# garg02/mpi-sppy

Measured on AMD Instinct MI355X. Metric: PH scenario-iterations/sec (farmer 100k) + time to conv<1e-4, higher is better.
Workload: dtype f64; 1 GPU; farmer crops_multiplier=1, 100000 scenarios (BASELINE configs[2]); scenarios=100000, scenarios_per_gpu=100000, n=12, m=7, nonants=3, parallelism=scenario-sharded x1, RCCL allreduce

## Files before the change

### mpi-sppy_amd/csrc/phx_jit.h

```cpp
#pragma once
#include <stdint.h>
#include <math.h>
#include <stdio.h>
#include <algorithm>
#include <sstream>
#include <string>
#include <vector>
#include "phx_setup.h"

namespace phx {

struct LaneStructure {
    int n = 0, m = 0, nnz = 0, npairs = 0, nvar = 0, nslot = 0;
    bool c_vary = false, bnd_vary = false, rhs_vary = false;
    bool scaled = false;
    std::vector<int32_t> row, col, kvar, col_slot;
    std::vector<int32_t> pair_a, pair_b, pair_pos;
    std::vector<uint8_t> lnz;
    std::vector<uint8_t> rfirst, cfirst, rempty, cempty;
    std::vector<uint8_t> lfin, ufin, fixed, blfin, bufin, eq;
    std::vector<double> Ac, dc, dr, c, lb, ub, bl, bu;
    double ipm_xs = 1.0, ipm_zs = 1.0, ipm_ws = 1.0;
    double multi_theta = 0.0;
    int multi_rounds = 0;
// ... 241 lines not shown
         "  phx_lane::lane_stamp(io, 1);\n"
         "  const int t = blockIdx.x * 64 + threadIdx.x;\n"
         "  bool still = false;\n"
         "  if (t < io.S) {\n"
         "    phx_lane::lane_stamp(io, 2);\n"
         "    still = " + wl + "(io, t);\n"
         "  }\n"
         "  phx_lane::lane_stamp(io, 3);\n"
         "  phx_lane::compact_lane(still, t, io.lanes_out, io.count_out);\n"
         "  phx_lane::lane_stamp(io, 4);\n"
         "  phx_lane::lane_stamp(io, 5);\n"
         "}\n";
    o << "extern \"C\" __global__ void __launch_bounds__(64, 1) phx_lane_warm_fz1(phx_lane::LaneIO io) {\n"
         "  phx_lane::warm_fused<PT>(io);\n"
         "}\n";
    o << "extern \"C\" __global__ void __launch_bounds__(64, 2) phx_lane_warm_fzr2(phx_lane::LaneIO io) {\n"
         "  phx_lane::warm_fused<PT, PHX_FZR2_CARRY_DEF, PHX_FZR2_PARK_DEF>(io);\n"
         "}\n";
    o << "extern \"C\" __global__ void __launch_bounds__(64, 1) phx_lane_all(phx_lane::LaneIO io, int rescue) {\n"
         "  if (phx_lane::gated(io.gate)) return;\n"
         "  phx_lane::zero_next_counts(io.counts_next);\n"
         "  const int t = blockIdx.x * 64 + threadIdx.x;\n"
         "  bool still = false;\n"
         "  if (t < io.S) still = phx_lane::all_lane<PT>(io, t, rescue);\n"
         "  phx_lane::compact_lane(still, t, io.lanes_out, io.count_out);\n"
         "}\n";
    o << "extern \"C\" __global__ void __launch_bounds__(64, 1) phx_lane_all_rl(phx_lane::LaneIO io, int rescue) {\n"
         "  if (phx_lane::gated(io.gate)) return;\n"
         "  phx_lane::zero_next_counts(io.counts_next);\n"
         "  const int t = blockIdx.x * 64 + threadIdx.x;\n"
         "  bool still = false;\n"
         "  if (t < io.S) still = phx_lane::all_lane<PT, false>(io, t, rescue);\n"
         "  phx_lane::compact_lane(still, t, io.lanes_out, io.count_out);\n"
         "}\n";
    o << "extern \"C\" __global__ void __launch_bounds__(64, 1) phx_lane_all_pk(phx_lane::LaneIO io, int rescue) {\n"
         "  __shared__ double pk[phx_lane::Data<PT>::PARK * 64];\n"
         "  if (phx_lane::gated(io.gate)) return;\n"
         "  phx_lane::zero_next_counts(io.counts_next);\n"
         "  const int t = blockIdx.x * 64 + threadIdx.x;\n"
         "  bool still = false;\n"
         "  if (t < io.S) still = phx_lane::all_lane<PT, false, true>(io, t, rescue, pk);\n"
         "  phx_lane::compact_lane(still, t, io.lanes_out, io.count_out);\n"
         "}\n";
    o << "extern \"C\" __global__ void __launch_bounds__(64) phx_fz_tail(phx_lane::LaneIO io, phx_lane::TailCopy tc) {\n"
         "  phx_lane::fz_tail<PT>(io, tc);\n"
         "}\n";
    o << "extern \"C\" __global__ void __launch_bounds__(64, 4) phx_lane_map(phx_lane::LaneIO io) {\n"
         "  if (phx_lane::gated(io.gate)) return;\n"
         "  phx_lane::zero_next_counts(io.counts_next);\n"
         "  const int t = blockIdx.x * 64 + threadIdx.x;\n"
         "  bool still = false;\n"
         "  if (t < io.S) still = phx_lane::map_lane<PT>(io, t);\n"
         "  phx_lane::compact_lane(still, t, io.lanes_out, io.count_out);\n"
         "}\n";
    const std::string wlr = with_map ? "phx_lane::warm_lane<PT, true, true>" : "phx_lane::warm_lane<PT, false, true>";
    o << "#ifdef PHX_LIST_RELOAD\n#define PHX_LIST_WAVES " << warm_waves << "\n#define PHX_LIST_FN " << wl
      << "\n#else\n#define PHX_LIST_WAVES 1\n#define PHX_LIST_FN " << wlr << "\n#endif\n";
    o << "extern \"C\" __global__ void __launch_bounds__(64, PHX_LIST_WAVES"
      << ") phx_lane_warm_list(phx_lane::LaneIO io, const int* lanes, const int* count) {\n"
// ... 59 lines not shown
```

### mpi-sppy_amd/csrc/phx_kernels.hip

```cpp
#include <hip/hip_runtime.h>
#include <stdio.h>
#include <string.h>
#include <math.h>
#include <string>
#include <vector>
#include <algorithm>
#include "../../include/phx.h"
#include "phx_core.h"
#include "phx_setup.h"
#include "phx_wg.h"
#include "phx_sp.h"
#include "phx_jit.h"
#include "phx_lane.h"
#include <hip/hiprtc.h>
#include <rccl/rccl.h>
#include <map>
#include <memory>
#include <mutex>
#include <stdlib.h>
#include <atomic>
#include <chrono>

#include "phx_lane_src.inc"

// ... 781 lines not shown
    int lane_ww = 2, lane_cw = 1;
    std::string lane_defs;
    LaneMod mod_ph, mod_fix;
    bool fix_built = false;
    bool fix_ok = false;
    bool fix_lane = false;
    double *fix_lb = nullptr, *fix_ub = nullptr;
    bool ovr_base_ok = false;
    const double* fix_vals = nullptr;
    const int32_t* fix_idx = nullptr;
    LaneMod mod_sub;
    std::vector<uint8_t> sub_mask;
    bool sub_ok = false;
    bool sub_lane = false;
    std::string sub_info;
    mutable std::string jit_text;
    const int32_t* fix_where = nullptr;
    const double *raw_lb = nullptr, *raw_ub = nullptr;
    int64_t raw_si = 0, raw_ss = 0;
    int32_t* fixer_new = nullptr;
    int32_t* donor_dev = nullptr;
    int donor_cap = 0;
    std::vector<int32_t> donor_lo, donor_hi;
    const void* donor_key[3] = {nullptr, nullptr, nullptr};
    int donor_key_n[2] = {0, 0};
    const double *ph_W = nullptr, *ph_rho = nullptr, *ph_xbar = nullptr;
    const int32_t* ph_idx = nullptr;
    int32_t ph_W_on = 0, ph_prox_on = 0;
    bool ph_dirty = false;
    int32_t* counts = nullptr;
// ... 72 lines not shown
#define PHX_CHECK(ctx, expr)                                                      \
    do {                                                                          \
        hipError_t _e = (expr);                                                   \
        if (_e != hipSuccess) {                                                   \
            (ctx)->err = std::string(#expr) + ": " + hipGetErrorString(_e);       \
            return 1;                                                             \
        }                                                                         \
    } while (0)

#define PHX_REQUIRE(ctx, cond, msg)                                               \
    do {                                                                          \
        if (!(cond)) { (ctx)->err = (msg); return 1; }                            \
    } while (0)

static inline unsigned nblk(int64_t n, int b) { return (unsigned)((n + b - 1) / b); }

static int ev_index(const phx_ctx* c, hipEvent_t e) {
    const hipEvent_t evs[5] = {c->ev0, c->ev1, c->ev2, c->ev3, c->ev4};
    for (int k = 0; k < 5; ++k)
        if (e && e == evs[k]) return k;
    return -1;
}

static hipError_t ev_record(phx_ctx* c, hipEvent_t e, hipStream_t st) {
    const hipError_t r = hipEventRecord(e, st);
    const int k = ev_index(c, e);
    if (r == hipSuccess && k >= 0) c->run.ev_rec |= 1u << k;
    return r;
}

// ... 544 lines not shown
                {
                    const size_t NS = (size_t)std::max(ctx->N, 1) * S;
                    ctx->lane_zero_d = ctx->alloc<double>(NS);
                    ctx->lane_zero_i = ctx->alloc<int32_t>(NS);
                    PHX_REQUIRE(ctx, ctx->lane_zero_d != nullptr && ctx->lane_zero_i != nullptr,
                                "phx_set_problem: out of device memory (lane stand-ins)");
                    PHX_CHECK(ctx, hipMemset(ctx->lane_zero_d, 0, sizeof(double) * NS));
                    PHX_CHECK(ctx, hipMemset(ctx->lane_zero_i, 0, sizeof(int32_t) * NS));
                }
                ctx->seed_buf = ctx->alloc<int32_t>(2 * SEED_T + 2);
                ctx->seed_aset = ctx->alloc<uint32_t>((size_t)SEED_T * phx_lane::aset_words(n, m));
                PHX_REQUIRE(ctx, ctx->aset != nullptr && ctx->seed_buf != nullptr,
                            "phx_set_problem: out of device memory (aset)");
                PHX_CHECK(ctx, hipMemset(ctx->aset, 0, sizeof(uint32_t) * nw));
                if (getenv("PHX_LANE_STAMPS") && atoi(getenv("PHX_LANE_STAMPS")) == 1) {
                    const size_t ns = (size_t)nblk(S, PHX_BLOCK) * 8;
                    ctx->lane_stamps = ctx->alloc<uint64_t>(ns);
                    if (ctx->lane_stamps) PHX_CHECK(ctx, hipMemset(ctx->lane_stamps, 0, sizeof(uint64_t) * ns));
                }
                if (want_map) {
                    ctx->lane_map = ctx->alloc<double>(mw * S);
                    PHX_REQUIRE(ctx, ctx->lane_map != nullptr, "phx_set_problem: out of device memory (map)");
                }
            }
        } else {
            ctx->jit_info = "off: " + why;
        }
    }
    hipLaunchKernelGGL(k_norm_init, dim3(nblk(S, PHX_BLOCK)), dim3(PHX_BLOCK), 0, 0, St, S);
    if (launch_begin(ctx, 0, 0, nullptr)) return 1;
    PHX_CHECK(ctx, hipGetLastError());
// ... 715 lines not shown
    io.status_out = status_out; io.iters_out = iters_out;
    io.max_it = o->ipm_max_it; io.ipm_tol = o->lane_ipm_tol > 0 ? o->lane_ipm_tol : o->ipm_tol; io.kkt_tol = o->kkt_tol; io.reg = o->reg;
    io.refine = o->refine_steps;
    io.as_rounds = o->as_rounds > 0 ? o->as_rounds : 1;
    io.single_after = 3;
    io.gate = gate;
    io.map = ctx->lane_map;
    io.fz = phx_lane::FusedW{};
    io.counts_next = nullptr;
    io.stamps = ctx->lane_stamps;
    return io;
}

static void report_lane_stamps(phx_ctx* ctx) {
    if (!ctx->lane_stamps) return;
    const unsigned G = nblk(ctx->S, PHX_BLOCK);
    std::vector<uint64_t> h((size_t)G * 8);
    if (hipMemcpy(h.data(), ctx->lane_stamps, sizeof(uint64_t) * h.size(), hipMemcpyDeviceToHost) != hipSuccess)
        return;
    uint64_t t0 = ~0ull, tend = 0, last_start = 0, first_end = ~0ull;
    double ph[5] = {0, 0, 0, 0, 0}, life = 0.0, lmax = 0.0;
    int nw = 0;
    for (unsigned b = 0; b < G; ++b) {
        const uint64_t* s = h.data() + (size_t)b * 8;
        if (!s[0] || !s[5] || s[5] < s[0]) continue;
        t0 = std::min(t0, s[0]);
        tend = std::max(tend, s[5]);
        last_start = std::max(last_start, s[0]);
        first_end = std::min(first_end, s[5]);
        for (int k = 0; k < 5; ++k) ph[k] += (double)(s[k + 1] - s[k]);
        life += (double)(s[5] - s[0]);
// ... 26 lines not shown
            const uint64_t* s = h.data() + (size_t)b * 8;
            if (!s[0] || !s[5] || s[5] < s[0] || s[5] < s[4]) continue;
            arr.emplace_back(s[4], b);
        }
        std::sort(arr.begin(), arr.end());
        const size_t n = arr.size(), nl = std::min<size_t>(n, 8);
        double ep_all = 0.0, ep_last = 0.0;
        for (size_t i = 0; i < n; ++i) {
            const uint64_t* s = h.data() + (size_t)arr[i].second * 8;
            ep_all += (double)(s[5] - s[4]);
            if (i + nl >= n) ep_last = std::max(ep_last, (double)(s[5] - s[4]));
        }
        if (n) {
            const uint64_t* sl = h.data() + (size_t)arr[n - 1].second * 8;
            fprintf(stderr,
                    "[lane stamps] by arrival at the epilogue: last arrival +%.2f us (block %u), its epilogue %.2f us; "
                    "launch end %.2f us after the last arrival; epilogue mean %.2f us, longest among the last %d "
                    "arrivals %.2f us\n",
                    (arr[n - 1].first - t0) * 0.01, arr[n - 1].second, (sl[5] - sl[4]) * 0.01,
                    (tend - arr[n - 1].first) * 0.01, ep_all / n * 0.01, (int)nl, ep_last * 0.01);
        }
    }
    fprintf(stderr,
            "[lane stamps] waves %d span %.2f us, last start +%.2f us, first end +%.2f us; per wave lifetime "
            "%.2f us (max %.2f): prologue %.2f, update_w %.2f, solve %.2f, compact %.2f, epilogue %.2f us\n",
            nw, (tend - t0) * 0.01, (last_start - t0) * 0.01, (first_end - t0) * 0.01, life / nw * 0.01, lmax * 0.01,
            ph[0] / nw * 0.01, ph[1] / nw * 0.01, ph[2] / nw * 0.01, ph[3] / nw * 0.01, ph[4] / nw * 0.01);
    (void)hipMemset(ctx->lane_stamps, 0, sizeof(uint64_t) * h.size());
}

static int rescue_rounds(const phx_solve_opts* o) {
// ... 44 lines not shown
        void* wargs[] = {&io};
        PHX_CHECK(ctx, hipModuleLaunchKernel(ctx->lane_warm_fn, G, 1, 1, PHX_BLOCK, 1, 1, 0, st, wargs, nullptr));
    }
    PHX_CHECK(ctx, hipGetLastError());
    io.counts_next = nullptr;
    io.lanes_out = ctx->lanesB;
    io.count_out = C + 1;
    io.as_rounds = std::max(io.as_rounds, rescue_rounds(o));
    const int32_t* in_l = ctx->lanesA;
    const int32_t* in_c = C;
    if (launch_cold(ctx, io, in_l, in_c, Gl, st)) return 1;
    *npass_out = 1;
    return 0;
}

static hipFunction_t fused_kernel(const phx_ctx* ctx, unsigned G) {
    static const bool fzr2_off = getenv("PHX_FZR2") && atoi(getenv("PHX_FZR2")) == 0;
    return (!fzr2_off && (int64_t)G > (int64_t)ctx->simds) ? ctx->lane_warm_fzr2_fn : ctx->lane_warm_fz1_fn;
}

static int enqueue_lane_solve(phx_ctx* ctx, const phx_solve_opts* o, hipStream_t st, int32_t* C, double* x_out,
                              double* y_out, double* obj_out, int32_t* status_out, int32_t* iters_out,
                              const int32_t* gate, hipEvent_t ev_a, hipEvent_t ev_b, hipEvent_t ev_c,
                              int* npass_out, unsigned cold_blocks = 0,
                              const phx_lane::FusedW* fz = nullptr, int mode = 0) {
    const int S = ctx->S;
    const unsigned G = nblk(S, PHX_BLOCK);
    phx_lane::LaneIO io = lane_io(ctx, o, x_out, y_out, obj_out, status_out, iters_out, gate);
    io.fz = fz ? *fz : phx_lane::FusedW{};
    if (fz) io.xbar_node = fz->stage;
    const bool warm_as = ctx->have_aset && o->as_rounds > 0 && ctx->lane_warm_fn;
    const bool use_map = ctx->lane_map != nullptr && ctx->lane_map_fn != nullptr;
    int npass = warm_as ? (use_map ? 2 : std::max(1, std::min(o->warm_passes, 8))) : 0;
// ... 11 lines not shown
        PHX_CHECK(ctx, hipModuleLaunchKernel(ctx->lane_all_fn, G, 1, 1, PHX_BLOCK, 1, 1, 0, st, aargs, nullptr));
        if (ev_b) PHX_CHECK(ctx, ev_record(ctx, ev_b, st));
        *npass_out = 0;
        return 0;
    }
    const unsigned Gl = std::min<unsigned>(G, 1024u);
    const unsigned Gc = cold_blocks ? std::min<unsigned>(G, cold_blocks) : Gl;
    if (ev_a) PHX_CHECK(ctx, ev_record(ctx, ev_a, st));
    for (int k = 0; k < npass && mode != 2; ++k) {
        io.lanes_out = L[k & 1]; io.count_out = C + k;
        io.counts_next = k == 0 ? next : nullptr;
        io.warm_rounds = use_map ? (k == 0 ? 0 : o->as_rounds) : (npass > 1 ? 1 : o->as_rounds);
        if (k == 0) {
            void* wargs[] = {&io};
            hipFunction_t fn = use_map ? ctx->lane_map_fn : (fz ? fused_kernel(ctx, G) : ctx->lane_warm_fn);
            PHX_CHECK(ctx, hipModuleLaunchKernel(fn, G, 1, 1, PHX_BLOCK, 1, 1, 0, st, wargs, nullptr));
            if (ev_b) PHX_CHECK(ctx, ev_record(ctx, ev_b, st));
        } else {
            const int32_t* in_l = L[(k - 1) & 1];
            const int32_t* in_c = C + k - 1;
            void* largs[] = {&io, &in_l, &in_c};
            PHX_CHECK(ctx, hipModuleLaunchKernel(ctx->lane_warm_list_fn, Gl, 1, 1, PHX_BLOCK, 1, 1, 0, st,
                                                 largs, nullptr));
        }
    }
    if (npass == 0 && ev_b) PHX_CHECK(ctx, ev_record(ctx, ev_b, st));
    *npass_out = npass;
    if (mode == 1) return 0;

    io.fz = phx_lane::FusedW{};
    if (mode == 2) io.xbar_node = ctx->ph_xbar;
// ... 580 lines not shown
        return 1;
    }
    ctx->comm_ranks = nranks;
    ctx->comm_rank = rank;
    return 0;
}

int phx_last_solve_stats(const phx_ctx* ctx, phx_solve_stats* out) {
    if (!ctx || !out) return 1;
    *out = ctx->stats;
    return 0;
}

const char* phx_jit_info(const phx_ctx* ctx) {
    if (!ctx) return "null context";
    ctx->jit_text = ctx->jit_info + ctx->sub_info;
    return ctx->jit_text.c_str();
}

int phx_debug_spd_inverse(const double* s_host, int32_t ma, double* inv_host) {
    if (!s_host || !inv_host || ma < 1 || ma > WG_BLK_MAX) return -1;
    const int ld = ma | 1;
    double* d = nullptr;
    int32_t* f = nullptr;
    if (hipMalloc(&d, sizeof(double) * (size_t)ma * ld) != hipSuccess) return -1;
    if (hipMalloc(&f, sizeof(int32_t)) != hipSuccess) { (void)hipFree(d); return -1; }
    std::vector<double> h((size_t)ma * ld, 0.0);
    for (int i = 0; i < ma; ++i)
        for (int j = 0; j <= i; ++j) h[(size_t)i * ld + j] = s_host[(size_t)i * ma + j];
    int rc = 0;
    if (hipMemcpy(d, h.data(), sizeof(double) * h.size(), hipMemcpyHostToDevice) != hipSuccess) rc = -1;
// ... 337 lines not shown
        fprintf(stderr, "[iterk] S=%d lane_mode=%d wg=%d sp=%d fused=%d (fz_env %d tail %d warm %d nnodes %d NNS %d N %d "
                "ntiles %d cover %d gseg %d segs_ok %d stage_len %d need %d W %d rho %d map %d passes %d as_rounds %d) "
                "depth %d max_iters %d\n", S, (int)lane_mode, (int)wg_mode, (int)sp_mode, (int)fused, (int)fz_env,
                ctx->lane_tail_fn != nullptr, ctx->lane_warm_fn != nullptr, T->nnodes, NNS, ctx->N, T->ntiles,
                T->nnodes_cover, gseg, (int)segs_ok, a->node_stage_len, 2 * NNS + 1 + a->conv_R,
                (int)(ctx->ph_W == a->W), (int)(ctx->ph_rho == a->rho), (int)use_map, o->warm_passes, o->as_rounds,
                depth, a->max_iters);
    struct OutSet { double *x, *y, *obj; int32_t *status, *iters; };
    OutSet X[2] = {{a->x, a->y, a->obj, a->status, a->iters}, {}};
    if (fused) {
        X[1] = OutSet{ctx->alt_x, a->y ? ctx->alt_y : nullptr, ctx->alt_obj, a->status ? ctx->alt_status : nullptr,
                      a->iters ? ctx->alt_iters : nullptr};
    } else {
        X[1] = X[0];
    }
    auto make_fz = [&](int k, bool first) {
        phx_lane::FusedW f{};
        f.on = 1;
        f.iter = k;
        f.first = first ? 1 : 0;
        f.from_shards = (!first && !multi) ? 1 : 0;
        f.fold_top = multi ? 1 : 0;
        f.nb = (int32_t)nblk(S, PHX_BLOCK);
        f.stage = stage;
        f.node_sums = a->node_sums;
        f.nns = NNS;
        f.x_prev = X[(k - 1) & 1].x;
        f.pc = a->prob_coeff;
        f.ctl = ctx->ctl;
        f.prog = ctx->prog_dev;
        f.part = ctx->fz_part;
        f.tk = ctx->tickets + 2 * TICKET_SET;
        f.g = gseg;
        f.R = a->conv_R;
        f.cnt = ctx->conv_cnt_dev;
        f.thresh = a->convthresh;
        return f;
    };
// ... 178 lines not shown
                        phx_lane::TailCopy tc{};
                        if (!tail_enq) {
                            tc.left_dst = (int32_t*)ctx->tail_dev;
                            tc.left_src = C;
                            if (a->seg_sums) {
                                tc.seg_dst = a->seg_sums;
                                tc.seg_src = stage + 2 * NNS + 1;
                                tc.nseg = a->conv_R;
                            }
                        }
                        if (iter0_exp && !adopt_pending && !iter0_exp_copied) {
                            tc.exp_dst = ctx->tail_dev + 1;
                            tc.exp_src = a->iter0_expect;
                        }
                        void* targs[] = {&tio, &tc};
                        PHX_CHECK(ctx, hipModuleLaunchKernel(ctx->lane_tail_fn, 1, 1, 1, PHX_BLOCK, 1, 1, 0, st,
                                                             targs, nullptr));
                        if (tc.left_dst) {
                            tail_enq = left_in_tail = true;
                            if (tc.seg_dst) seg_copied = true;
                        }
                        if (tc.exp_dst) iter0_exp_copied = exp_in_tail = true;
                    }
                    enq.push_back(Enq{C, npass, false});
                    k_enq = k;
                    continue;
                }
                const OutSet& xin = X[(k - 1) & 1];
                const OutSet& xout = X[k & 1];
                if (small_xw) {
                    IterkCtl ic{};
                    ic.ctl = ctx->ctl;
// ... 282 lines not shown
```

### mpi-sppy_amd/csrc/phx_lane.h

```cpp
#pragma once
#if !defined(__HIPCC_RTC__)
#include <stdint.h>
#include <math.h>
#if defined(__HIPCC__)
#include <hip/hip_runtime.h>
#endif
#else
typedef long long int64_t;
typedef int int32_t;
typedef unsigned int uint32_t;
typedef unsigned long long uint64_t;
#endif

#if defined(__HIPCC__) || defined(__HIPCC_RTC__)
#define PHX_LD __host__ __device__ __forceinline__
#define PHX_UNROLL _Pragma("unroll")
#define PHX_NOUNROLL _Pragma("nounroll")
#else
#define PHX_LD inline
#define PHX_UNROLL
#define PHX_NOUNROLL
#endif
#ifdef PHX_IPM_PASS_ROLLED
#define PHX_IPM_PASS_LOOP PHX_NOUNROLL
// ... 54 lines not shown
constexpr int32_t FLAG_WRITTEN = 2;
constexpr int32_t FLAG_MAP = 4;

struct IterkProgress {
    uint64_t word;
    double conv;
};

struct FusedW {
    int32_t on;
    int32_t iter;
    int32_t first;
    int32_t from_shards;
    int32_t fold_top;
    int32_t nb;
    double* stage;
    double* node_sums;
    int32_t nns;
    const double* x_prev;
    const double* pc;
    int32_t* ctl;
    IterkProgress* prog;
    double* part;
    unsigned int* tk;
    int32_t g, R;
    const double* cnt;
    double thresh;
};

struct LaneIO {
// ... 43 lines not shown
    FusedW fz;
    uint64_t* stamps;
};

struct TailCopy {
    int32_t* left_dst;
    const int32_t* left_src;
    double* seg_dst;
    const double* seg_src;
    int32_t nseg;
    double* exp_dst;
    const double* exp_src;
};

#if defined(__HIPCC__) || defined(__HIPCC_RTC__)
__device__ __forceinline__ void lane_stamp(const LaneIO& io, int k) {
    if (io.stamps && threadIdx.x == 0) io.stamps[(uint64_t)blockIdx.x * 8 + k] = wall_clock64();
}
#endif

#if (defined(__HIPCC__) || defined(__HIPCC_RTC__)) && !defined(PHX_OUT_PLAIN)
#define PHX_OUT(lv, v) __hip_atomic_store(&(lv), (v), __ATOMIC_RELAXED, __HIP_MEMORY_SCOPE_AGENT)
#else
#define PHX_OUT(lv, v) ((lv) = (v))
#endif

PHX_LD bool gated(const int32_t* gate) { return gate && *(const volatile int32_t*)gate; }

PHX_LD void opaque(double& v) {
#if defined(__HIP_DEVICE_COMPILE__) || defined(__HIPCC_RTC__)
    __asm__ volatile("" : "+v"(v));
#else
// ... 1549 lines not shown
            *(volatile int32_t*)f.ctl = 1;
        }
        publish_progress(f.prog, it, done ? 1 : 0, conv);
    }
    return done;
}

__device__ __forceinline__ double* fz_part_set(const FusedW& f, int np, int it) {
    return f.part + (int64_t)(it & 1) * ((int64_t)f.nb + TICKET_SHARDS) * np;
}
template <int NP>
__device__ __forceinline__ void fz_shard_load(const FusedW& f, int it, double* r) {
    const unsigned nsh = (unsigned)f.nb < TICKET_SHARDS ? (unsigned)f.nb : TICKET_SHARDS;
    const double* sp = fz_part_set(f, NP, it) + (int64_t)f.nb * NP;
    PHX_UNROLL for (int u = 0; u < (TICKET_SHARDS * NP + 63) / 64; ++u) {
        const unsigned i = 64u * u + threadIdx.x;
        r[u] = i < nsh * NP ? load_wt(sp + i) : 0.0;
    }
}
template <int NP>
__device__ __forceinline__ double fz_shard_sum(const double* r, int e) {
    double a = 0.0;
    PHX_UNROLL for (int q = 0; q < TICKET_SHARDS; ++q) a += lane_get(r[(q * NP + e) / 64], (q * NP + e) % 64);
    return a;
}
template <class PT>
__device__ __forceinline__ void fz_inputs(const FusedW& f, const double* sv, double* in) {
    constexpr int NS = PT::nslot() > 0 ? PT::nslot() : 1;
    constexpr int NP = 2 * NS + 2;
    if (f.from_shards) {
        PHX_UNROLL for (int e = 0; e < NP; ++e) in[e] = fz_shard_sum<NP>(sv, e);
    } else {
        PHX_UNROLL for (int e = 0; e < NP; ++e) in[e] = 0.0;
        PHX_UNROLL for (int t = 0; t < PT::nslot(); ++t) {
            in[t] = f.stage[t];
            in[NS + t] = f.stage[f.nns + t];
        }
        in[2 * NS] = f.stage[2 * f.nns + 1 + f.g];
        in[2 * NS + 1] = f.stage[2 * f.nns];
    }
}
template <int NS>
__device__ __forceinline__ void fz_store_stage(const FusedW& f, const double* in) {
    PHX_UNROLL for (int t = 0; t < NS; ++t) {
        f.stage[t] = in[t];
        f.stage[f.nns + t] = in[NS + t];
// ... 85 lines not shown
    const int e = threadIdx.x;
    if (e < NV) {
        double a = 0.0;
        for (unsigned q = 0; q < nsh; ++q) a += load_wt(&shard_part[q * NP + e]);
        if (e < NS) f.stage[e] = a;
        else if (e < 2 * NS) f.stage[f.nns + (e - NS)] = a;
        else {
            for (int r = 0; r < f.R; ++r) f.stage[2 * f.nns + 1 + r] = r == f.g ? a : 0.0;
            f.stage[2 * f.nns] =
                (double)__hip_atomic_load(io.count_out, __ATOMIC_RELAXED, __HIP_MEMORY_SCOPE_AGENT);
        }
    }
}

template <class PT>
__device__ void fz_tail(const LaneIO& io, const TailCopy& tc) {
    const FusedW& f = io.fz;
    constexpr int NS = PT::nslot() > 0 ? PT::nslot() : 1;
    constexpr int NP = 2 * NS + 2;
    double sv[(TICKET_SHARDS * NP + 63) / 64], in[NP];
    fz_shard_load<NP>(f, f.iter, sv);
    const bool run = !gated(io.gate);
    const bool fold = run && !f.fold_top;
    PHX_UNROLL for (int e = 0; e < NP; ++e) in[e] = fz_shard_sum<NP>(sv, e);
    if (fold) {
        if (threadIdx.x == 0) fz_store_stage<NS>(f, in);
        if (tc.seg_dst)
            for (int g = threadIdx.x; g < tc.nseg; g += (int)blockDim.x) tc.seg_dst[g] = g == f.g ? in[2 * NS] : 0.0;
    }
    tail_copy(tc, !fold);
    if (!run) return;
    (void)fz_decide(f, f.iter, fz_conv(f, in[2 * NS], fold ? nullptr : f.stage + 2 * f.nns + 1));
}

template <class PT>
__device__ void seed_block(const LaneIO& io, const int32_t* tl, int T, const uint32_t* tmpl) {
    constexpr int NC = seed_coords<PT>();
    constexpr int TS = seed_templates_staged<PT>() > 0 ? seed_templates_staged<PT>() : 1;
    constexpr int NCP = NC > 0 ? NC : 1;
// ... 38 lines not shown
    for (int w = 0; w < nw; ++w) io.aset[(int64_t)w * io.S + sc] = tmpl[(int64_t)best * nw + w];
}

__device__ __forceinline__ void zero_next_counts(int32_t* next) {
    if (next && blockIdx.x == 0 && threadIdx.x < 16) next[threadIdx.x] = 0;
}

__device__ __forceinline__ void compact_lane(bool still, int sc, int32_t* out, int32_t* count) {
    const unsigned long long b = __ballot(still);
    const int lane = threadIdx.x & 63;
    int base = 0;
    if (lane == 0 && b) base = atomicAdd(count, (int32_t)__popcll(b));
    base = __shfl(base, 0, 64);
    if (still) out[base + __popcll(b & ((1ull << lane) - 1ull))] = sc;
}
template <class PT, bool CARRY = PHX_CARRY_DEF, bool PARK = false>
__device__ __forceinline__ void warm_fused(const LaneIO& io) {
    const FusedW& f = io.fz;
    constexpr int NS = PT::nslot() > 0 ? PT::nslot() : 1;
    constexpr int NP = 2 * NS + 2;
    constexpr int NVA = PT::NMAX_V, NW = aset_words(PT::NMAX_N, PT::NMAX_M);
    const int sc = blockIdx.x * 64 + threadIdx.x;
    const bool live = sc < io.S;
    const int s = live ? sc : 0;
    const int64_t S = io.S;
    double av[NVA], xv[NS], wv[NS], rv[NS], pcv[NS];
    uint32_t aw[NW];
    PHX_UNROLL for (int v = 0; v < PT::nvar(); ++v) av[v] = io.Av[(int64_t)v * S + s];
    PHX_UNROLL for (int k = 0; k < aset_words(PT::n(), PT::m()); ++k) aw[k] = io.aset[(int64_t)k * S + s];
    PHX_UNROLL for (int j = 0; j < PT::n(); ++j) {
        const int t = PT::col_slot(j);
        if (t >= 0) {
            const int64_t o = (int64_t)t * S + s;
            xv[t] = f.x_prev[(int64_t)j * S + s];
            wv[t] = io.W[o];
            rv[t] = io.rho[o];
            pcv[t] = f.pc[o];
        }
    }
    double sv[(TICKET_SHARDS * NP + 63) / 64], in[NP];
    fz_shard_load<NP>(f, f.iter - 1, sv);
    lane_stamp(io, 0);
    if (gated(io.gate)) return;
    fz_inputs<PT>(f, sv, in);
    if (!fz_prologue<PT>(io, in)) return;
    zero_next_counts(io.counts_next);
    lane_stamp(io, 1);
    double xb[NS], dl = 0.0;
    PHX_UNROLL for (int t = 0; t < PT::nslot(); ++t) {
        xb[t] = in[t];
        const double diff = xv[t] - xb[t];
        wv[t] = wv[t] + rv[t] * diff;
        if (live) PHX_OUT(const_cast<double*>(io.W)[(int64_t)t * S + sc], wv[t]);
        dl += fabs(diff);
    }
    lane_stamp(io, 2);
#ifndef PHX_FZ_NO_LDS_KEEP
    __shared__ double fz_keep[(NS + 1) * 64];
    PHX_UNROLL for (int t = 0; t < PT::nslot(); ++t) fz_keep[t * 64 + threadIdx.x] = pcv[t];
    fz_keep[NS * 64 + threadIdx.x] = dl;
#endif
    bool still = false;
    double xn[NS];
    if (live) {
        ASet<PT> a;
        aset_from_words<PT>(aw, a);
        double xp[PT::NMAX_N], z[PT::NMAX_M];
        PHX_UNROLL for (int j = 0; j < PT::n(); ++j) xp[j] = 0.0;
        PHX_UNROLL for (int i = 0; i < PT::m(); ++i) z[i] = 0.0;
        int c;
        if (PARK) {
            __shared__ double fz_park[Data<PT>::PARK * 64];
            {
                const Data<PT> D0(io, sc, av, wv, rv, xb);
                D0.park(fz_park, threadIdx.x);
                c = io.warm_rounds > 0 ? as_round<PT, CARRY, true>(io, D0, a, xp, z, 0) : 2;
            }
            int nr = 1;
            PHX_NOUNROLL for (int r = 1; r < io.warm_rounds && c == 1; ++r, ++nr) {
                const Data<PT> Dr(io, sc, fz_park, threadIdx.x);
                c = as_round<PT, CARRY, true>(io, Dr, a, xp, z, r);
            }
            if (io.stamps) {
                int wmax = 0;
                for (int q = 1; q <= 8; ++q) wmax = __ballot(nr >= q) ? q : wmax;
                if (threadIdx.x == 0) io.stamps[(uint64_t)blockIdx.x * 8 + 6] = (uint64_t)wmax;
            }
            if (c == 2) PHX_LANE_STAT(3);
            if (c == 0) {
                const Data<PT> Dw(io, sc, fz_park, threadIdx.x);
                write_certified<PT>(io, Dw, sc, a, xp, z, 0);
            }
        } else {
            const Data<PT> D0(io, sc, av, wv, rv, xb);
            c = io.warm_rounds > 0 ? as_round<PT, CARRY>(io, D0, a, xp, z, 0) : 2;
            int nr = 1;
            PHX_NOUNROLL for (int r = 1; r < io.warm_rounds && c == 1; ++r, ++nr) c = as_round<PT, CARRY>(io, D0, a, xp, z, r);
            if (io.stamps) {
                int wmax = 0;
                for (int q = 1; q <= 8; ++q) wmax = __ballot(nr >= q) ? q : wmax;
                if (threadIdx.x == 0) io.stamps[(uint64_t)blockIdx.x * 8 + 6] = (uint64_t)wmax;
            }
            if (c == 2) PHX_LANE_STAT(3);
            if (c == 0) write_certified<PT>(io, D0, sc, a, xp, z, 0);
        }
        if (c != 0) {
            aset_store<PT>(io, sc, a);
            io.status[sc] = 0;
            io.flags[sc] = 0;
            still = true;
        } else {
            PHX_UNROLL for (int j = 0; j < PT::n(); ++j)
                if (PT::col_slot(j) >= 0) xn[PT::col_slot(j)] = xp[j] * (PT::scaled() ? PT::dcs(j) : 1.0);
        }
    }
    double v[NP];
    PHX_UNROLL for (int e = 0; e < NP; ++e) v[e] = 0.0;
#ifndef PHX_FZ_NO_LDS_KEEP
    PHX_UNROLL for (int t = 0; t < PT::nslot(); ++t) pcv[t] = fz_keep[t * 64 + threadIdx.x];
    dl = fz_keep[NS * 64 + threadIdx.x];
#endif
    if (live) {
        v[2 * NS] = dl;
        if (!still)
            PHX_UNROLL for (int t = 0; t < PT::nslot(); ++t) {
                const double w = pcv[t] * xn[t];
                v[t] += w;
                v[NS + t] += w * xn[t];
            }
    }
    lane_stamp(io, 3);
    compact_lane(still, sc, io.lanes_out, io.count_out);
    v[2 * NS + 1] = (double)__popcll(__ballot(still));
    lane_stamp(io, 4);
    fz_fold<PT>(io, v);
    lane_stamp(io, 5);
}

#endif

}
```

Baseline: 4.226 billion scenario-iterations/s.

## Add block-level fused fold with 256-thread blocks for the fzr2 warm kernel

The fzr2 fused warm kernel now runs with 256-thread blocks. Per-wave LDS buffers move to dynamic shared memory. When the block count is small enough, the cross-scenario reduction writes one partial per block, which the next launch and the tail kernel read and sum, replacing the sharded ticket-based fold. This targets the cost of the per-wave atomic or ticket fold and its serialization. In exchange it uses more LDS per block, adds a __syncthreads, and constrains occupancy through launch bounds (256,2).

```diff
diff --git a/mpi-sppy_amd/csrc/phx_jit.h b/mpi-sppy_amd/csrc/phx_jit.h
--- a/mpi-sppy_amd/csrc/phx_jit.h
+++ b/mpi-sppy_amd/csrc/phx_jit.h
@@ -279,8 +279,8 @@
     o << "extern \"C\" __global__ void __launch_bounds__(64, 1) phx_lane_warm_fz1(phx_lane::LaneIO io) {\n"
          "  phx_lane::warm_fused<PT>(io);\n"
          "}\n";
-    o << "extern \"C\" __global__ void __launch_bounds__(64, 2) phx_lane_warm_fzr2(phx_lane::LaneIO io) {\n"
-         "  phx_lane::warm_fused<PT, PHX_FZR2_CARRY_DEF, PHX_FZR2_PARK_DEF>(io);\n"
+    o << "extern \"C\" __global__ void __launch_bounds__(256, 2) phx_lane_warm_fzr2(phx_lane::LaneIO io) {\n"
+         "  phx_lane::warm_fused<PT, PHX_FZR2_CARRY_DEF, PHX_FZR2_PARK_DEF, true>(io);\n"
          "}\n";
     o << "extern \"C\" __global__ void __launch_bounds__(64, 1) phx_lane_all(phx_lane::LaneIO io, int rescue) {\n"
          "  if (phx_lane::gated(io.gate)) return;\n"
@@ -307,7 +307,7 @@
          "  if (t < io.S) still = phx_lane::all_lane<PT, false, true>(io, t, rescue, pk);\n"
          "  phx_lane::compact_lane(still, t, io.lanes_out, io.count_out);\n"
          "}\n";
-    o << "extern \"C\" __global__ void __launch_bounds__(64) phx_fz_tail(phx_lane::LaneIO io, phx_lane::TailCopy tc) {\n"
+    o << "extern \"C\" __global__ void __launch_bounds__(256) phx_fz_tail(phx_lane::LaneIO io, phx_lane::TailCopy tc) {\n"
          "  phx_lane::fz_tail<PT>(io, tc);\n"
          "}\n";
     o << "extern \"C\" __global__ void __launch_bounds__(64, 4) phx_lane_map(phx_lane::LaneIO io) {\n"
diff --git a/mpi-sppy_amd/csrc/phx_kernels.hip b/mpi-sppy_amd/csrc/phx_kernels.hip
--- a/mpi-sppy_amd/csrc/phx_kernels.hip
+++ b/mpi-sppy_amd/csrc/phx_kernels.hip
@@ -819,6 +819,9 @@
     bool sub_ok = false;
     bool sub_lane = false;
     std::string sub_info;
+    mutable hipFunction_t fzr2_static_fn = nullptr;
+    mutable int fzr2_static_lds = 0;
+    std::string fz_info;
     mutable std::string jit_text;
     const int32_t* fix_where = nullptr;
     const double *raw_lb = nullptr, *raw_ub = nullptr;
@@ -921,6 +924,7 @@
     } while (0)
 
 static inline unsigned nblk(int64_t n, int b) { return (unsigned)((n + b - 1) / b); }
+static inline unsigned stamp_rows(int64_t S) { return nblk(S, 256) * 4u; }
 
 static int ev_index(const phx_ctx* c, hipEvent_t e) {
     const hipEvent_t evs[5] = {c->ev0, c->ev1, c->ev2, c->ev3, c->ev4};
@@ -1495,7 +1499,7 @@
                             "phx_set_problem: out of device memory (aset)");
                 PHX_CHECK(ctx, hipMemset(ctx->aset, 0, sizeof(uint32_t) * nw));
                 if (getenv("PHX_LANE_STAMPS") && atoi(getenv("PHX_LANE_STAMPS")) == 1) {
-                    const size_t ns = (size_t)nblk(S, PHX_BLOCK) * 8;
+                    const size_t ns = (size_t)stamp_rows(S) * 8;
                     ctx->lane_stamps = ctx->alloc<uint64_t>(ns);
                     if (ctx->lane_stamps) PHX_CHECK(ctx, hipMemset(ctx->lane_stamps, 0, sizeof(uint64_t) * ns));
                 }
@@ -2241,7 +2245,7 @@
 
 static void report_lane_stamps(phx_ctx* ctx) {
     if (!ctx->lane_stamps) return;
-    const unsigned G = nblk(ctx->S, PHX_BLOCK);
+    const unsigned G = stamp_rows(ctx->S);
     std::vector<uint64_t> h((size_t)G * 8);
     if (hipMemcpy(h.data(), ctx->lane_stamps, sizeof(uint64_t) * h.size(), hipMemcpyDeviceToHost) != hipSuccess)
         return;
@@ -2298,7 +2302,7 @@
         if (n) {
             const uint64_t* sl = h.data() + (size_t)arr[n - 1].second * 8;
             fprintf(stderr,
-                    "[lane stamps] by arrival at the epilogue: last arrival +%.2f us (block %u), its epilogue %.2f us; "
+                    "[lane stamps] by arrival at the epilogue: last arrival +%.2f us (wave %u), its epilogue %.2f us; "
                     "launch end %.2f us after the last arrival; epilogue mean %.2f us, longest among the last %d "
                     "arrivals %.2f us\n",
                     (arr[n - 1].first - t0) * 0.01, arr[n - 1].second, (sl[5] - sl[4]) * 0.01,
@@ -2373,9 +2377,41 @@
     return 0;
 }
 
+static size_t fused_lds_bytes(const phx_ctx* ctx, unsigned waves) {
+    const LaneStructure& L = *ctx->lane_L;
+    const int NS = std::max(L.nslot, 1), PARK = std::max(L.nvar, 1) + 2 * NS + 1;
+    return (size_t)waves * (NS + 1 + PARK) * 64 * sizeof(double);
+}
+static bool fused_lds_fits(const phx_ctx* ctx, unsigned waves) {
+    if (!ctx->lane_L || !ctx->lane_warm_fzr2_fn) return false;
+    if (ctx->fzr2_static_fn != ctx->lane_warm_fzr2_fn) {
+        int stat = 0;
+        if (hipFuncGetAttribute(&stat, HIP_FUNC_ATTRIBUTE_SHARED_SIZE_BYTES, ctx->lane_warm_fzr2_fn) != hipSuccess) {
+            stat = 4096;
+            (void)hipGetLastError();
+            if (getenv("PHX_ITERK_DEBUG"))
+                fprintf(stderr, "[iterk] phx_lane_warm_fzr2: static LDS size not available, %d B assumed\n", stat);
+        }
+        ctx->fzr2_static_fn = ctx->lane_warm_fzr2_fn;
+        ctx->fzr2_static_lds = stat;
+    }
+    return (size_t)ctx->fzr2_static_lds + fused_lds_bytes(ctx, waves) <= 65536;
+}
 static hipFunction_t fused_kernel(const phx_ctx* ctx, unsigned G) {
     static const bool fzr2_off = getenv("PHX_FZR2") && atoi(getenv("PHX_FZR2")) == 0;
-    return (!fzr2_off && (int64_t)G > (int64_t)ctx->simds) ? ctx->lane_warm_fzr2_fn : ctx->lane_warm_fz1_fn;
+    return (!fzr2_off && (int64_t)G > (int64_t)ctx->simds && fused_lds_fits(ctx, 1)) ? ctx->lane_warm_fzr2_fn
+                                                                                     : ctx->lane_warm_fz1_fn;
+}
+static unsigned fused_block_fold(const phx_ctx* ctx, bool multi) {
+    const char* e = getenv("PHX_FZB");
+    const int force = e ? atoi(e) : -1;
+    if (multi || force == 0 || !fused_lds_fits(ctx, phx_lane::FZB_NT / 64)) return 0;
+    const unsigned G = nblk(ctx->S, PHX_BLOCK), B = nblk(ctx->S, phx_lane::FZB_NT);
+    if (force != 1 && fused_kernel(ctx, G) != ctx->lane_warm_fzr2_fn) return 0;
+    const char* l = getenv("PHX_FZB_LIMIT");
+    const int64_t limit = l ? atoll(l) : 4096, NP = 2 * std::max(ctx->N, 1) + 2;
+    if ((int64_t)B * NP > limit) return 0;
+    return B;
 }
 
 static int enqueue_lane_solve(phx_ctx* ctx, const phx_solve_opts* o, hipStream_t st, int32_t* C, double* x_out,
@@ -2417,7 +2453,14 @@
         if (k == 0) {
             void* wargs[] = {&io};
             hipFunction_t fn = use_map ? ctx->lane_map_fn : (fz ? fused_kernel(ctx, G) : ctx->lane_warm_fn);
-            PHX_CHECK(ctx, hipModuleLaunchKernel(fn, G, 1, 1, PHX_BLOCK, 1, 1, 0, st, wargs, nullptr));
+            if (fz && fz->fzb) {
+                PHX_CHECK(ctx, hipModuleLaunchKernel(ctx->lane_warm_fzr2_fn, (unsigned)fz->fzb, 1, 1, phx_lane::FZB_NT, 1, 1,
+                                                     (unsigned)fused_lds_bytes(ctx, phx_lane::FZB_NT / 64), st, wargs, nullptr));
+            } else {
+                const bool dyn = fz && !use_map && fn == ctx->lane_warm_fzr2_fn;
+                PHX_CHECK(ctx, hipModuleLaunchKernel(fn, G, 1, 1, PHX_BLOCK, 1, 1,
+                                                     dyn ? (unsigned)fused_lds_bytes(ctx, 1) : 0u, st, wargs, nullptr));
+            }
             if (ev_b) PHX_CHECK(ctx, ev_record(ctx, ev_b, st));
         } else {
             const int32_t* in_l = L[(k - 1) & 1];
@@ -3028,7 +3071,7 @@
 
 const char* phx_jit_info(const phx_ctx* ctx) {
     if (!ctx) return "null context";
-    ctx->jit_text = ctx->jit_info + ctx->sub_info;
+    ctx->jit_text = ctx->jit_info + ctx->sub_info + ctx->fz_info;
     return ctx->jit_text.c_str();
 }
 
@@ -3396,6 +3439,11 @@
     } else {
         X[1] = X[0];
     }
+    const unsigned fzb = fused ? fused_block_fold(ctx, multi) : 0u;
+    if (fused)
+        ctx->fz_info = fzb ? "; fused fold: blocks (" + std::to_string(fzb) + " x " + std::to_string(phx_lane::FZB_NT) + " threads)"
+                           : "; fused fold: shards (" + std::to_string(nblk(S, PHX_BLOCK)) + " x " +
+                                 std::to_string(PHX_BLOCK) + " threads)";
     auto make_fz = [&](int k, bool first) {
         phx_lane::FusedW f{};
         f.on = 1;
@@ -3404,6 +3452,7 @@
         f.from_shards = (!first && !multi) ? 1 : 0;
         f.fold_top = multi ? 1 : 0;
         f.nb = (int32_t)nblk(S, PHX_BLOCK);
+        f.fzb = (int32_t)fzb;
         f.stage = stage;
         f.node_sums = a->node_sums;
         f.nns = NNS;
@@ -3612,8 +3661,8 @@
                             tc.exp_src = a->iter0_expect;
                         }
                         void* targs[] = {&tio, &tc};
-                        PHX_CHECK(ctx, hipModuleLaunchKernel(ctx->lane_tail_fn, 1, 1, 1, PHX_BLOCK, 1, 1, 0, st,
-                                                             targs, nullptr));
+                        PHX_CHECK(ctx, hipModuleLaunchKernel(ctx->lane_tail_fn, 1, 1, 1, fzb ? phx_lane::FZB_NT : PHX_BLOCK, 1, 1,
+                                                             0, st, targs, nullptr));
                         if (tc.left_dst) {
                             tail_enq = left_in_tail = true;
                             if (tc.seg_dst) seg_copied = true;
diff --git a/mpi-sppy_amd/csrc/phx_lane.h b/mpi-sppy_amd/csrc/phx_lane.h
--- a/mpi-sppy_amd/csrc/phx_lane.h
+++ b/mpi-sppy_amd/csrc/phx_lane.h
@@ -92,6 +92,7 @@
     int32_t from_shards;
     int32_t fold_top;
     int32_t nb;
+    int32_t fzb;
     double* stage;
     double* node_sums;
     int32_t nns;
@@ -165,8 +166,11 @@
 };
 
 #if defined(__HIPCC__) || defined(__HIPCC_RTC__)
+__device__ __forceinline__ uint64_t stamp_row() {
+    return ((uint64_t)blockIdx.x * blockDim.x + threadIdx.x) >> 6;
+}
 __device__ __forceinline__ void lane_stamp(const LaneIO& io, int k) {
-    if (io.stamps && threadIdx.x == 0) io.stamps[(uint64_t)blockIdx.x * 8 + k] = wall_clock64();
+    if (io.stamps && (threadIdx.x & 63) == 0) io.stamps[stamp_row() * 8 + k] = wall_clock64();
 }
 #endif
 
@@ -1746,8 +1750,35 @@
     const unsigned nsh = (unsigned)f.nb < TICKET_SHARDS ? (unsigned)f.nb : TICKET_SHARDS;
     const double* sp = fz_part_set(f, NP, it) + (int64_t)f.nb * NP;
     PHX_UNROLL for (int u = 0; u < (TICKET_SHARDS * NP + 63) / 64; ++u) {
-        const unsigned i = 64u * u + threadIdx.x;
+        const unsigned i = 64u * u + (threadIdx.x & 63u);
         r[u] = i < nsh * NP ? load_wt(sp + i) : 0.0;
+    }
+}
+constexpr int FZB_NT = 256;
+template <int NP>
+__device__ __forceinline__ void fz_block_load(const FusedW& f, int it, double* a) {
+    const double* bp = fz_part_set(f, NP, it);
+    const unsigned B = (unsigned)f.fzb;
+    PHX_UNROLL for (int e = 0; e < NP; ++e) a[e] = 0.0;
+    for (unsigned b0 = threadIdx.x; b0 < B; b0 += 2u * FZB_NT) {
+        double l[2][NP];
+        PHX_UNROLL for (int u = 0; u < 2; ++u) {
+            const unsigned b = b0 + (unsigned)FZB_NT * u;
+            PHX_UNROLL for (int e = 0; e < NP; ++e) l[u][e] = b < B ? bp[(int64_t)e * B + b] : 0.0;
+        }
+        PHX_UNROLL for (int u = 0; u < 2; ++u) PHX_UNROLL for (int e = 0; e < NP; ++e) a[e] += l[u][e];
+    }
+}
+template <int NP>
+__device__ __forceinline__ void fz_block_sum(double* a, double* red) {
+    const int lane = threadIdx.x & 63, w = threadIdx.x >> 6;
+    PHX_UNROLL for (int e = 0; e < NP; ++e) a[e] = wave_sum(a[e]);
+    if (lane == 0) PHX_UNROLL for (int e = 0; e < NP; ++e) red[w * NP + e] = a[e];
+    __syncthreads();
+    PHX_UNROLL for (int e = 0; e < NP; ++e) {
+        double s = 0.0;
+        PHX_UNROLL for (int q = 0; q < FZB_NT / 64; ++q) s += red[q * NP + e];
+        a[e] = lane_get(s, 0);
     }
 }
 template <int NP>
@@ -1757,11 +1788,22 @@
     return a;
 }
 template <class PT>
-__device__ __forceinline__ void fz_inputs(const FusedW& f, const double* sv, double* in) {
+__device__ __forceinline__ void fz_entry_load(const FusedW& f, bool bfold, double* sv, double* in) {
+    constexpr int NP = 2 * (PT::nslot() > 0 ? PT::nslot() : 1) + 2;
+    if (!bfold) fz_shard_load<NP>(f, f.iter - 1, sv);
+    else if (f.from_shards) fz_block_load<NP>(f, f.iter - 1, in);
+}
+template <class PT>
+__device__ __forceinline__ void fz_entry_sum(const FusedW& f, bool bfold, double* in, double* red) {
+    constexpr int NP = 2 * (PT::nslot() > 0 ? PT::nslot() : 1) + 2;
+    if (bfold && f.from_shards) fz_block_sum<NP>(in, red);
+}
+template <class PT>
+__device__ __forceinline__ void fz_inputs(const FusedW& f, bool bfold, const double* sv, double* in) {
     constexpr int NS = PT::nslot() > 0 ? PT::nslot() : 1;
     constexpr int NP = 2 * NS + 2;
     if (f.from_shards) {
-        PHX_UNROLL for (int e = 0; e < NP; ++e) in[e] = fz_shard_sum<NP>(sv, e);
+        if (!bfold) PHX_UNROLL for (int e = 0; e < NP; ++e) in[e] = fz_shard_sum<NP>(sv, e);
     } else {
         PHX_UNROLL for (int e = 0; e < NP; ++e) in[e] = 0.0;
         PHX_UNROLL for (int t = 0; t < PT::nslot(); ++t) {
@@ -1877,15 +1919,35 @@
 }
 
 template <class PT>
+__device__ void fz_block_fold(const LaneIO& io, double* v, double* red) {
+    const FusedW& f = io.fz;
+    constexpr int NS = PT::nslot() > 0 ? PT::nslot() : 1;
+    constexpr int NV = 2 * NS + 1, NP = NV + 1;
+    PHX_UNROLL for (int e = 0; e < NV; ++e) v[e] = wave_sum(v[e]);
+    const int lane = threadIdx.x & 63, w = threadIdx.x >> 6;
+    if (lane == 0) PHX_UNROLL for (int e = 0; e < NP; ++e) red[w * NP + e] = v[e];
+    __syncthreads();
+    if (threadIdx.x < NP) {
+        const int e = threadIdx.x;
+        double a = 0.0;
+        PHX_UNROLL for (int q = 0; q < FZB_NT / 64; ++q) a += red[q * NP + e];
+        fz_part_set(f, NP, f.iter)[(int64_t)e * gridDim.x + blockIdx.x] = a;
+    }
+}
+
+template <class PT>
 __device__ void fz_tail(const LaneIO& io, const TailCopy& tc) {
     const FusedW& f = io.fz;
     constexpr int NS = PT::nslot() > 0 ? PT::nslot() : 1;
     constexpr int NP = 2 * NS + 2;
     double sv[(TICKET_SHARDS * NP + 63) / 64], in[NP];
-    fz_shard_load<NP>(f, f.iter, sv);
+    __shared__ double red[(FZB_NT / 64) * NP];
+    if (f.fzb) fz_block_load<NP>(f, f.iter, in);
+    else fz_shard_load<NP>(f, f.iter, sv);
     const bool run = !gated(io.gate);
     const bool fold = run && !f.fold_top;
-    PHX_UNROLL for (int e = 0; e < NP; ++e) in[e] = fz_shard_sum<NP>(sv, e);
+    if (f.fzb) fz_block_sum<NP>(in, red);
+    else PHX_UNROLL for (int e = 0; e < NP; ++e) in[e] = fz_shard_sum<NP>(sv, e);
     if (fold) {
         if (threadIdx.x == 0) fz_store_stage<NS>(f, in);
         if (tc.seg_dst)
@@ -1954,13 +2016,20 @@
     base = __shfl(base, 0, 64);
     if (still) out[base + __popcll(b & ((1ull << lane) - 1ull))] = sc;
 }
-template <class PT, bool CARRY = PHX_CARRY_DEF, bool PARK = false>
+template <class PT>
+__device__ __forceinline__ double* fz_wave_lds() {
+    extern __shared__ double fz_dyn[];
+    constexpr int NS = PT::nslot() > 0 ? PT::nslot() : 1;
+    return fz_dyn + (threadIdx.x >> 6) * ((NS + 1 + Data<PT>::PARK) * 64);
+}
+template <class PT, bool CARRY = PHX_CARRY_DEF, bool PARK = false, bool WIDE = false>
 __device__ __forceinline__ void warm_fused(const LaneIO& io) {
     const FusedW& f = io.fz;
     constexpr int NS = PT::nslot() > 0 ? PT::nslot() : 1;
     constexpr int NP = 2 * NS + 2;
     constexpr int NVA = PT::NMAX_V, NW = aset_words(PT::NMAX_N, PT::NMAX_M);
-    const int sc = blockIdx.x * 64 + threadIdx.x;
+    const int lane = threadIdx.x & 63;
+    const int sc = blockIdx.x * blockDim.x + threadIdx.x;
     const bool live = sc < io.S;
     const int s = live ? sc : 0;
     const int64_t S = io.S;
@@ -1979,10 +2048,13 @@
         }
     }
     double sv[(TICKET_SHARDS * NP + 63) / 64], in[NP];
-    fz_shard_load<NP>(f, f.iter - 1, sv);
+    __shared__ double fz_red[WIDE ? 2 * (FZB_NT / 64) * NP : 1];
+    const bool bfold = WIDE && f.fzb != 0;
+    fz_entry_load<PT>(f, bfold, sv, in);
     lane_stamp(io, 0);
+    fz_entry_sum<PT>(f, bfold, in, fz_red);
     if (gated(io.gate)) return;
-    fz_inputs<PT>(f, sv, in);
+    fz_inputs<PT>(f, bfold, sv, in);
     if (!fz_prologue<PT>(io, in)) return;
     zero_next_counts(io.counts_next);
     lane_stamp(io, 1);
@@ -1996,9 +2068,10 @@
     }
     lane_stamp(io, 2);
 #ifndef PHX_FZ_NO_LDS_KEEP
-    __shared__ double fz_keep[(NS + 1) * 64];
-    PHX_UNROLL for (int t = 0; t < PT::nslot(); ++t) fz_keep[t * 64 + threadIdx.x] = pcv[t];
-    fz_keep[NS * 64 + threadIdx.x] = dl;
+    __shared__ double fz_keep_s[WIDE ? 1 : (NS + 1) * 64];
+    double* const fz_keep = WIDE ? fz_wave_lds<PT>() : fz_keep_s;
+    PHX_UNROLL for (int t = 0; t < PT::nslot(); ++t) fz_keep[t * 64 + lane] = pcv[t];
+    fz_keep[NS * 64 + lane] = dl;
 #endif
     bool still = false;
     double xn[NS];
@@ -2010,25 +2083,26 @@
         PHX_UNROLL for (int i = 0; i < PT::m(); ++i) z[i] = 0.0;
         int c;
         if (PARK) {
-            __shared__ double fz_park[Data<PT>::PARK * 64];
+            __shared__ double fz_park_s[WIDE ? 1 : Data<PT>::PARK * 64];
+            double* const fz_park = WIDE ? fz_wave_lds<PT>() + (NS + 1) * 64 : fz_park_s;
             {
                 const Data<PT> D0(io, sc, av, wv, rv, xb);
-                D0.park(fz_park, threadIdx.x);
+                D0.park(fz_park, lane);
                 c = io.warm_rounds > 0 ? as_round<PT, CARRY, true>(io, D0, a, xp, z, 0) : 2;
             }
             int nr = 1;
             PHX_NOUNROLL for (int r = 1; r < io.warm_rounds && c == 1; ++r, ++nr) {
-                const Data<PT> Dr(io, sc, fz_park, threadIdx.x);
+                const Data<PT> Dr(io, sc, fz_park, lane);
                 c = as_round<PT, CARRY, true>(io, Dr, a, xp, z, r);
             }
             if (io.stamps) {
                 int wmax = 0;
                 for (int q = 1; q <= 8; ++q) wmax = __ballot(nr >= q) ? q : wmax;
-                if (threadIdx.x == 0) io.stamps[(uint64_t)blockIdx.x * 8 + 6] = (uint64_t)wmax;
+                if (lane == 0) io.stamps[stamp_row() * 8 + 6] = (uint64_t)wmax;
             }
             if (c == 2) PHX_LANE_STAT(3);
             if (c == 0) {
-                const Data<PT> Dw(io, sc, fz_park, threadIdx.x);
+                const Data<PT> Dw(io, sc, fz_park, lane);
                 write_certified<PT>(io, Dw, sc, a, xp, z, 0);
             }
         } else {
@@ -2039,7 +2113,7 @@
             if (io.stamps) {
                 int wmax = 0;
                 for (int q = 1; q <= 8; ++q) wmax = __ballot(nr >= q) ? q : wmax;
-                if (threadIdx.x == 0) io.stamps[(uint64_t)blockIdx.x * 8 + 6] = (uint64_t)wmax;
+                if (lane == 0) io.stamps[stamp_row() * 8 + 6] = (uint64_t)wmax;
             }
             if (c == 2) PHX_LANE_STAT(3);
             if (c == 0) write_certified<PT>(io, D0, sc, a, xp, z, 0);
@@ -2057,8 +2131,8 @@
     double v[NP];
     PHX_UNROLL for (int e = 0; e < NP; ++e) v[e] = 0.0;
 #ifndef PHX_FZ_NO_LDS_KEEP
-    PHX_UNROLL for (int t = 0; t < PT::nslot(); ++t) pcv[t] = fz_keep[t * 64 + threadIdx.x];
-    dl = fz_keep[NS * 64 + threadIdx.x];
+    PHX_UNROLL for (int t = 0; t < PT::nslot(); ++t) pcv[t] = fz_keep[t * 64 + lane];
+    dl = fz_keep[NS * 64 + lane];
 #endif
     if (live) {
         v[2 * NS] = dl;
@@ -2073,7 +2147,8 @@
     compact_lane(still, sc, io.lanes_out, io.count_out);
     v[2 * NS + 1] = (double)__popcll(__ballot(still));
     lane_stamp(io, 4);
-    fz_fold<PT>(io, v);
+    if (bfold) fz_block_fold<PT>(io, v, fz_red + (FZB_NT / 64) * NP);
+    else fz_fold<PT>(io, v);
     lane_stamp(io, 5);
 }
 
```

Result: faster. 4.384 billion scenario-iterations/s (median of 6 runs) (+3.7%).
